# LANL-Bioinformatics/PCRamp

Hardware: AMD Instinct MI355X
Metric: primer-pair x target amplification evals/sec (higher is better)
Workload: dtype u32

## Files before the change

pcramp_amd/csrc/pcr_device.hip:

```cpp
#include <hip/hip_runtime.h>
#include <cstring>
#include <rocprim/device/device_radix_sort.hpp>

#include <stdint.h>
#include <string.h>
#include <math.h>
#include <stdlib.h>
#include <string>
#include <vector>
#include <chrono>
#include <algorithm>
#include <unordered_map>
#include <type_traits>
#include <thread>
#include <mutex>
#include <condition_variable>
#include <functional>
#include <memory>

#include "../../include/pcramp_hip.h"
#include "pcr_host.hpp"

using pcrhost::Planes;

// ... 1188 lines not shown
		const bool vec_ok = ((uintptr_t)d_fr % 16 == 0) && ((uintptr_t)d_rf % 16 == 0) && (bits_bytes % 16 == 0);
		if(!vec_ok){
			HIP_TRY(hipMemsetAsync(d_fr, 0, bits_bytes, ctx->stream));
			HIP_TRY(hipMemsetAsync(d_rf, 0, bits_bytes, ctx->stream));
		}
		if((rc = vec_ok ? st.ship(d_fr, bits_bytes, d_rf, bits_bytes) : st.ship()) != PCR_OK) return rc;
	}
	timer.next(5);
	const uint32_t mask_words = (2*n_pairs + 31)/32;
	if((rc = ctx->mask.ensure((size_t)S.n_slots*mask_words)) != PCR_OK) return rc;
	if((rc = ctx->status.ensure(1)) != PCR_OK) return rc;
	const bool dev_n = S.n_touched == N_TOUCHED_UNKNOWN;
	const uint32_t *n_dev = dev_n ? S.ctrl.p + 3 : nullptr;
	const uint32_t n_t = dev_n ? 0u : S.n_touched, n_db = n_t*S.db_cap;
	const unsigned threads = dev_n ? 256 : 128;
	const unsigned grid = dev_n ? (unsigned)std::min<uint64_t>(((uint64_t)S.n*S.db_cap + threads - 1)/threads, 1024) : (n_db + threads - 1)/threads;
	const unsigned mgrid = dev_n ? std::min<unsigned>((S.n + MATCH_WAVES - 1)/MATCH_WAVES, 1024u) : (n_t + MATCH_WAVES - 1)/MATCH_WAVES;
	hipLaunchKernelGGL(k_match, dim3(std::max(mgrid, 1u)), dim3(64*MATCH_WAVES), 0, ctx->stream, S.db.p, n_t, n_dev, S.db_cap,
		S.touched.p, S.d_seg_hi, ctx->d_oligos, 2*n_pairs, mask_words, ctx->mask.p, ctx->status.p,
		prestaged ? fa->pub_counters : (const uint32_t *)nullptr, prestaged ? ctx->mail_dev + (fa->pub_seq % pcr_ctx::MAIL_RING) : (pcr_ctx::Mail *)nullptr,
		prestaged ? fa->pub_seq : 0u);
	HIP_TRY(hipGetLastError());
	hipLaunchKernelGGL(k_pair, dim3(grid), dim3(threads), 0, ctx->stream, S.db.p, n_db, n_dev, S.db_cap, S.touched.p, S.d_seg_hi, ctx->mask.p,
		mask_words, ctx->d_oligos, n_pairs, S.planes.p, S.d_blk_off.p, S.d_len.p, S.d_active.p, a->amp_min, a->amp_max,
		a->ident_threshold, a->use_taq_mama, d_fr, d_rf, words, ctx->status.p);
	HIP_TRY(hipGetLastError());
	return PCR_OK;
}

template<int NSLOT, int KLO>
int launch_scan2_nw(pcr_ctx *ctx, SeqSet &S, uint32_t nw, uint32_t group0, uint32_t n_groups, uint32_t gw, uint32_t ncand, const HitSink &sink,
	const uint32_t *d_tab, const uint32_t *d_bias, const uint32_t *tile_ids, uint32_t n_tiles, const uint32_t *orient_ids)
{
#define SCAN2_ARGS S.nib.p, S.planes.p, S.valid_d(), S.d_blk_off.p, S.d_len.p, S.d_active.p, S.tile_seq.p, S.tile_pos0.p, \
	d_tab, d_bias, group0, gw, tile_ids, orient_ids, ctx->d_cand_fwd, ctx->d_cand_rc, ctx->d_cand_floor, ncand, sink
	const dim3 grid(n_tiles, n_groups), block(SCAN2_THREADS);
	switch(nw){
		case 1: hipLaunchKernelGGL((k_scan2<1, NSLOT, KLO>), grid, block, 0, ctx->stream, SCAN2_ARGS); break;
		case 2: hipLaunchKernelGGL((k_scan2<2, NSLOT, KLO>), grid, block, 0, ctx->stream, SCAN2_ARGS); break;
		case 3: hipLaunchKernelGGL((k_scan2<3, NSLOT, KLO>), grid, block, 0, ctx->stream, SCAN2_ARGS); break;
		case 4: hipLaunchKernelGGL((k_scan2<4, NSLOT, KLO>), grid, block, 0, ctx->stream, SCAN2_ARGS); break;
		case 5: hipLaunchKernelGGL((k_scan2<5, NSLOT, KLO>), grid, block, 0, ctx->stream, SCAN2_ARGS); break;
		case 6: hipLaunchKernelGGL((k_scan2<6, NSLOT, KLO>), grid, block, 0, ctx->stream, SCAN2_ARGS); break;
		case 7: hipLaunchKernelGGL((k_scan2<7, NSLOT, KLO>), grid, block, 0, ctx->stream, SCAN2_ARGS); break;
		default: hipLaunchKernelGGL((k_scan2<8, NSLOT, KLO>), grid, block, 0, ctx->stream, SCAN2_ARGS); break;
	}
#undef SCAN2_ARGS
// ... 1001 lines not shown
					if(ctx->debug_log) fprintf(stderr, "[pcramp] k_seed: %d workgroups per CU x %u CUs\n", per_cu, ctx->n_cu);
#define SEED_ARGS S.tb_d(), S.planes.p, S.valid_d(), S.d_blk_off.p, S.d_nblk_real.p, S.d_len.p, S.d_active.p, S.tile_seq.p, S.tile_pos0.p, \
	S.tile_degen.p, S.n_tiles, ST, ctx->d_cand_fwd, ctx->d_cand_rc, ctx->d_cand_floor, ncand, IA, sgrid.x, sink
					if(cand_lds) hipLaunchKernelGGL(k_seed<true>, fgrid, sblock, dyn, ctx->stream, SEED_ARGS);
					else hipLaunchKernelGGL(k_seed<false>, fgrid, sblock, dyn, ctx->stream, SEED_ARGS);
#undef SEED_ARGS
					HIP_TRY(hipGetLastError());
					if(need_seedset && (rc = launch_scan2(ctx, S, tab_seedset, ncand, sink, d_tab_seedset, d_bias_seedset, S.degen_tiles.p,
						S.n_degen_tiles, d_map_seedset)) != PCR_OK) return rc;
				}
			}
			scan_prof.finish();
		}
		if(n_live && !irr_fused){
			const unsigned irr_grid = (n_live + IRR_THREADS*IRR_PER_LANE - 1)/(IRR_THREADS*IRR_PER_LANE);
			hipLaunchKernelGGL(k_scan_irr, dim3(irr_grid), dim3(IRR_THREADS), 0, ctx->stream, S.irr.p, S.irr_perm.p, n_live,
				S.d_active.p, ctx->d_cand_fwd, ctx->d_cand_floor, ncand, sink);
			HIP_TRY(hipGetLastError());
		}
		if(async && fa && fa->staged && (cap == POST_CAP || cap == 128 || cap == 256) && 2*fa->n_pairs <= 32*POST_MASK_WORDS){
			++ctx->mail_seq;
			const uint64_t bw = (S.n + 63)/64;
#define POST_ARGS ctx->hits.p, d_seq_count, ctx->best.p, ncand, S.planes.p, S.d_blk_off.p, S.irr.p, S.irr_off.p, S.db.p, S.d_seg_hi, d_counters, ctx->epoch, S.n, \
	fa->d_oligos, fa->n_pairs, (2*fa->n_pairs + 31)/32, S.d_len.p, S.d_active.p, fa->a->amp_min, fa->a->amp_max, \
	fa->a->ident_threshold, fa->a->use_taq_mama, fa->d_fr, fa->d_rf, bw, ctx->mail_dev + (ctx->mail_seq % pcr_ctx::MAIL_RING), ctx->mail_seq
			if(cap == POST_CAP){
				static const int post_waves = getenv("PCRAMP_POST_WAVES") ? atoi(getenv("PCRAMP_POST_WAVES")) : 8;
				if(post_waves == 16) hipLaunchKernelGGL(k_post<16>, dim3((S.n + 15)/16), dim3(1024), 0, ctx->stream, POST_ARGS);
				else if(post_waves == 4) hipLaunchKernelGGL(k_post<4>, dim3((S.n + 3)/4), dim3(256), 0, ctx->stream, POST_ARGS);
				else hipLaunchKernelGGL(k_post<8>, dim3((S.n + 7)/8), dim3(512), 0, ctx->stream, POST_ARGS);
				S.ctrl_clean = true; S.touched_from_seg = true;
			}
			else if(cap == 128) hipLaunchKernelGGL((k_post_big<128, 4>), dim3((S.n + 3)/4), dim3(256), 0, ctx->stream, POST_ARGS);
			else hipLaunchKernelGGL((k_post_big<256, 4>), dim3((S.n + 3)/4), dim3(256), 0, ctx->stream, POST_ARGS);
#undef POST_ARGS
			HIP_TRY(hipGetLastError());
			fa->posted = true;
			S.db_cap = cap; S.n_slots = n_slots;
			S.n_touched = N_TOUCHED_UNKNOWN; S.n_entries = 1; S.have_db = true; S.touched_built = false;
			return PCR_OK;
		}
		hipLaunchKernelGGL(k_touched, dim3((S.n + 255)/256), dim3(256), 0, ctx->stream, d_seq_count, S.n, d_counters, S.touched.p);
		HIP_TRY(hipGetLastError());
		S.touched_built = true;
		uint32_t np2 = 1; while(np2 < cap) np2 <<= 1;
#define FIN_ARGS ctx->hits.p, d_seq_count, cap, ctx->best.p, ncand, S.planes.p, S.d_blk_off.p, S.irr.p, S.irr_off.p, S.db.p, S.d_seg_hi, \
	d_counters, ctx->epoch, S.touched.p
// ... 397 lines not shown
```

pcramp_amd/csrc/pcr_entry_sw_thermo.inc:

```
namespace {

int word_codes(const Planes &w, uint8_t *codes)
{
	const int len = pcrhost::planes_size(w), start = pcrhost::planes_start(w);
	for(int k = 0;k < 32;++k) codes[k] = (k < len && start + k < 32) ? (uint8_t)pcrhost::planes_nibble(w, start + k) : 0;
	return len;
}

void pair_queries(const pcr_pair *pairs, uint32_t n_pairs, std::vector<uint8_t> &q, std::vector<uint8_t> &ql, std::vector<BgPairDev> &bp)
{
	q.assign((size_t)n_pairs*4*32, 0); ql.assign((size_t)n_pairs*4, 0); bp.assign(n_pairs, BgPairDev());
	for(uint32_t p = 0;p < n_pairs;++p){
		const Planes F = pcrhost::planes_of_word(pairs[p].f.w), R = pcrhost::planes_of_word(pairs[p].r.w);
		const Planes o[4] = {F, pcrhost::planes_revcomp(F), R, pcrhost::planes_revcomp(R)};
		uint8_t last[4][2];
		for(int l = 0;l < 4;++l){
			ql[(size_t)p*4 + l] = (uint8_t)word_codes(o[l], &q[((size_t)p*4 + l)*32]);
			const int stop = pcrhost::planes_stop(o[l]);
			last[l][0] = (stop >= 1) ? (uint8_t)pcrhost::planes_nibble(o[l], stop - 1) : 0;
			last[l][1] = (stop >= 0) ? (uint8_t)pcrhost::planes_nibble(o[l], stop) : 0;
		}
		BgPairDev b;
		float f_norm = 2.0f*(unsigned)pcrhost::planes_size(F), r_norm = 2.0f*(unsigned)pcrhost::planes_size(R);
		if(f_norm > 0.0f) f_norm = 1.0f/f_norm;
// ... 200 lines not shown
	int rc;
	const float thr2 = collect_threshold*collect_threshold;
	std::vector<OligoDev> ol(2*(size_t)n_pairs);
	for(uint32_t i = 0;i < n_pairs;++i){ fill_oligo(ol[2*i], pairs[i].f.w, thr2); fill_oligo(ol[2*i + 1], pairs[i].r.w, thr2); }
	if((rc = ctx->oligos.ensure(ol.size())) != PCR_OK) return rc;
	HIP_TRY(hipMemcpyAsync(ctx->oligos.p, ol.data(), ol.size()*sizeof(OligoDev), hipMemcpyHostToDevice, ctx->stream));
	HIP_TRY(hipStreamSynchronize(ctx->stream));
	const uint32_t mask_words = (2*n_pairs + 31)/32;
	if((rc = ctx->mask.ensure((size_t)S.n_slots*mask_words)) != PCR_OK) return rc;
	if((rc = ctx->status.ensure(1)) != PCR_OK) return rc;
	if((rc = ctx->counters.ensure(4)) != PCR_OK) return rc;
	const unsigned threads = 128;
	const uint32_t n_db = S.n_touched*S.db_cap;
	const unsigned grid = (n_db + threads - 1)/threads;
	hipLaunchKernelGGL(k_match, dim3((S.n_touched + MATCH_WAVES - 1)/MATCH_WAVES), dim3(64*MATCH_WAVES), 0, ctx->stream, S.db.p, S.n_touched, (const uint32_t *)nullptr, S.db_cap,
		S.touched.p, S.d_seg_hi, ctx->oligos.p, 2*n_pairs, mask_words, ctx->mask.p, (uint32_t *)nullptr, (const uint32_t *)nullptr, (pcr_ctx::Mail *)nullptr, 0u);
	HIP_TRY(hipGetLastError());
	uint32_t n_amp = 0, status = 0;
	for(int attempt = 0;;++attempt){
		if((rc = ctx->amp_recs.ensure(ctx->amp_cap)) != PCR_OK) return rc;
		HIP_TRY(hipMemsetAsync(ctx->counters.p, 0, 4*sizeof(uint32_t), ctx->stream));
		HIP_TRY(hipMemsetAsync(ctx->status.p, 0, sizeof(uint32_t), ctx->stream));
		hipLaunchKernelGGL(k_pair_emit, dim3(grid), dim3(threads), 0, ctx->stream, S.db.p, n_db, S.db_cap, S.touched.p, S.d_seg_hi, ctx->mask.p, mask_words,
			ctx->oligos.p, n_pairs, S.planes.p, S.d_blk_off.p, S.d_len.p, S.d_active.p, amp_min, amp_max,
			ctx->amp_recs.p, (uint32_t)ctx->amp_cap, ctx->counters.p, ctx->status.p);
		HIP_TRY(hipGetLastError());
		HIP_TRY(hipMemcpyAsync(&n_amp, ctx->counters.p, sizeof(uint32_t), hipMemcpyDeviceToHost, ctx->stream));
		HIP_TRY(hipMemcpyAsync(&status, ctx->status.p, sizeof(uint32_t), hipMemcpyDeviceToHost, ctx->stream));
		HIP_TRY(hipStreamSynchronize(ctx->stream));
		if(n_amp <= ctx->amp_cap) break;
		if(attempt >= 4 || n_amp > (1u << 29)){ g_err = "candidate amplicon list does not fit"; return PCR_ERR_CAPACITY; }
		ctx->amp_cap = (size_t)n_amp + (n_amp >> 3);
	}
	if(status & 1u){ g_err = "Sequence::has_split: range is out of bounds"; return PCR_ERR_RANGE; }
	*n_amp_out = n_amp;
	return PCR_OK;
}

static int background_match_ordered(pcr_ctx *ctx, SeqSet &S, const pcr_pair *pairs, uint32_t n_pairs, const pcr_background_args *args, uint64_t *bits)
{
	const uint64_t words = (S.n + 63)/64;
	const size_t total = (size_t)n_pairs*words;
	int rc;
	uint32_t n_amp = 0;
	if((rc = candidate_amplicons(ctx, S, pairs, n_pairs, args->collect_threshold, args->amp_min, args->amp_max, &n_amp)) != PCR_OK) return rc;
	if((rc = upload_pair_queries(ctx, pairs, n_pairs)) != PCR_OK) return rc;
	if((rc = ctx->bits_fr.ensure(total)) != PCR_OK) return rc;
// ... 496 lines not shown
```

pcramp_amd/csrc/pcr_screen.inc:

```
__device__ __forceinline__ bool db_slot(uint32_t g, uint32_t n, uint32_t cap, const uint32_t *__restrict__ touched,
	const uint32_t *__restrict__ seg_hi, uint32_t &slot)
{
	if(g >= n) return false;
	const uint32_t seq = touched[g/cap];
	slot = seq*cap + g % cap;
	return slot < seg_hi[seq];
}

constexpr int MATCH_WAVES = 4;
__global__ __launch_bounds__(64*MATCH_WAVES) void k_match(const DevEntry *__restrict__ db, uint32_t n_touched, const uint32_t *__restrict__ n_touched_dev, uint32_t cap,
	const uint32_t *__restrict__ touched, const uint32_t *__restrict__ seg_hi, const OligoDev *__restrict__ oligos, uint32_t n_oligo,
	uint32_t mask_words, uint32_t *__restrict__ mask, uint32_t *__restrict__ status,
	const uint32_t *__restrict__ pub_counters, PassMail *pub_mail, uint32_t pub_seq)
{
	if(blockIdx.x == 0 && threadIdx.x == 0 && status) status[0] = 0;
	if(pub_mail && blockIdx.x == 0 && threadIdx.x < 64){
		if(threadIdx.x < 4) pub_mail->counters[threadIdx.x] = pub_counters[threadIdx.x];
		__threadfence_system();
		__builtin_amdgcn_wave_barrier();
		if(threadIdx.x == 0) __hip_atomic_store((uint32_t *)&pub_mail->seq, pub_seq, __ATOMIC_RELEASE, __HIP_MEMORY_SCOPE_SYSTEM);
	}
	if(n_touched_dev) n_touched = *n_touched_dev;
	const uint32_t lane = threadIdx.x & 63u, sub = lane >> 5, ol = lane & 31u;
	for(uint32_t t_idx = blockIdx.x*MATCH_WAVES + (threadIdx.x >> 6);t_idx < n_touched;t_idx += gridDim.x*MATCH_WAVES){
// ... 56 lines not shown
			const float corr = fminf(1.0f, c_taq_mama[16*(4*taq_idx(t2) + taq_idx(t1)) + (4*taq_idx(o.p2) + taq_idx(o.p1))]);
			id = __fmul_rn(id, corr);
		}
	}
	return id;
}

__device__ bool has_split(const uint4 *__restrict__ planes, uint64_t base, int32_t start, int32_t n)
{
	int32_t pos = start;
	const int32_t end = start + n;
	while(pos < end){
		const uint32_t b = (uint32_t)pos >> 5, sh = (uint32_t)pos & 31;
		const uint4 v = planes[base + b];
		uint32_t nz = (v.x | v.y | v.z | v.w) >> sh;
		const int32_t span = min(32 - (int32_t)sh, end - pos);
		const uint32_t want = (span == 32) ? 0xFFFFFFFFu : ((1u << span) - 1u);
		if((nz & want) != want) return true;
		pos += span;
	}
	return false;
}

__global__ void k_pair(const DevEntry *__restrict__ db, uint32_t n, const uint32_t *__restrict__ n_touched_dev, uint32_t cap, const uint32_t *__restrict__ touched,
	const uint32_t *__restrict__ seg_hi, const uint32_t *__restrict__ mask, uint32_t mask_words, const OligoDev *__restrict__ oligos, uint32_t n_pairs,
	const uint4 *__restrict__ planes, const uint64_t *__restrict__ blk_off, const uint64_t *__restrict__ len,
	const uint8_t *__restrict__ active, int32_t amp_min, int32_t amp_max, float ident_thr, int use_taq,
	uint64_t *__restrict__ bits_fr, uint64_t *__restrict__ bits_rf, uint64_t bit_words, uint32_t *__restrict__ status)
{
	if(n_touched_dev) n = (*n_touched_dev)*cap;
	for(uint32_t t = blockIdx.x*blockDim.x + threadIdx.x;t < n;t += gridDim.x*blockDim.x){
	uint32_t i;
	if(!db_slot(t, n, cap, touched, seg_hi, i)) continue;
	const DevEntry ei = db[i];
	if(ei.strand != 1) continue;
	if(!active[ei.seq]) continue;
	const uint32_t hi = seg_hi[ei.seq];
	const int32_t L = (int32_t)len[ei.seq];
	const uint64_t base = blk_off[ei.seq];
	for(uint32_t j = i + 1;j < hi;++j){
		const DevEntry ej = db[j];
		if(ej.loc - ei.loc > amp_max + 128) break;
		if(ej.strand != 2) continue;
		for(uint32_t w = 0;w < mask_words;++w){
			const uint32_t mi = mask[(size_t)i*mask_words + w], mj = mask[(size_t)j*mask_words + w];
			uint32_t fr = mi & (mj >> 1) & 0x55555555u;
			uint32_t rf = (mi >> 1) & mj & 0x55555555u;
			uint32_t any = fr | rf;
			while(any){
				const uint32_t bit = __ffs(any) - 1;
				any &= any - 1;
				const uint32_t pair = (w*32 + bit) >> 1;
				if(pair >= n_pairs) break;
				const OligoDev F = oligos[2*pair], R = oligos[2*pair + 1];
				for(int orient = 0;orient < 2;++orient){
					if(!(((orient == 0) ? fr : rf) >> bit & 1u)) continue;
					const OligoDev &P = (orient == 0) ? F : R;
					const OligoDev &M = (orient == 0) ? R : F;
					if(ei.loc + P.stop >= ej.loc - M.stop) continue;
					int32_t amp_start = ei.loc + P.start;
					const int32_t amp_stop = min(ej.loc - M.start, L - 1);
					int32_t amp_len = amp_stop - amp_start + 1;
					if(amp_len < amp_min || amp_len > amp_max) continue;
					if(amp_start < 0){ amp_len += amp_start; amp_start = 0; }
					if(amp_len < 0 || amp_start + amp_len > L){ atomicOr(status, 1u); continue; }
					if(has_split(planes, base, amp_start, amp_len)) continue;
					const float f = identity(F, (orient == 0) ? ei.w : ej.w, use_taq);
					const float r = identity(R, (orient == 0) ? ej.w : ei.w, use_taq);
					if(sqrtf(__fmul_rn(f, r)) >= ident_thr){
						uint64_t *dst = (orient == 0) ? bits_fr : bits_rf;
						atomicOr((unsigned long long *)&dst[(size_t)pair*bit_words + (ei.seq >> 6)], 1ull << (ei.seq & 63));
					}
				}
			}
		}
	}
	}
}

__global__ void k_pair_moves(const DevEntry *__restrict__ db, uint32_t n, uint32_t cap, const uint32_t *__restrict__ touched,
	const uint32_t *__restrict__ seg_hi, const uint32_t *__restrict__ mask, const OligoDev *__restrict__ base ,
	const OligoDev *__restrict__ variants, uint32_t n_variants, int side,
	const uint4 *__restrict__ planes, const uint64_t *__restrict__ blk_off, const uint64_t *__restrict__ len,
	const uint8_t *__restrict__ active, const uint8_t *__restrict__ has_eos, int32_t amp_min, int32_t amp_max, float ident_thr, int use_taq,
	uint64_t *__restrict__ bits_fr, uint64_t *__restrict__ bits_rf, uint64_t bit_words, uint32_t *__restrict__ status)
{
	const uint32_t t = blockIdx.x*blockDim.x + threadIdx.x;
	uint32_t e;
	if(!db_slot(t, n, cap, touched, seg_hi, e)) return;
// ... 102 lines not shown
			if(iloc + P.stop >= jloc - M.stop) continue;
			int32_t amp_start = iloc + P.start;
			const int32_t amp_stop = min(jloc - M.start, L - 1);
			int32_t amp_len = amp_stop - amp_start + 1;
			if(amp_len < amp_min || amp_len > amp_max) continue;
			if(amp_start < 0){ amp_len += amp_start; amp_start = 0; }
			if(amp_len < 0 || amp_start + amp_len > L){ atomicOr(status, 1u); continue; }
			if(eos && has_split(planes, blk_base, amp_start, amp_len)) continue;
			best = fmaxf(best, r.id);
		}
		if(best < 0.0f) continue;
		uint64_t *dst = (orient == 0) ? bits_fr : bits_rf;
		const uint64_t bit = 1ull << (seq & 63);
		for(uint32_t v = 0;v < n_variants;++v){
			const float var = identity(variants[v], ee.w, use_taq);
			const float f = (side == 0) ? var : best, r2 = (side == 0) ? best : var;
			if(sqrtf(__fmul_rn(f, r2)) >= ident_thr)
				atomicOr((unsigned long long *)&dst[(size_t)v*bit_words + (seq >> 6)], bit);
		}
	}
}

constexpr uint32_t POST_CAP = 64, POST_MASK_WORDS = 4;
struct PostEnt { Planes w; int32_t loc; uint32_t strand; };
template<int POST_WAVES>
struct PostShared {
	OligoDev ol[32*POST_MASK_WORDS];
	uint64_t keys[POST_WAVES][POST_CAP]; PostEnt ent[POST_WAVES][POST_CAP]; uint32_t msk[POST_WAVES][POST_CAP][POST_MASK_WORDS];
};

template<int POST_WAVES>
__global__ __launch_bounds__(64*POST_WAVES) void k_post(const Hit *__restrict__ hits, uint32_t *__restrict__ seq_count,
	const uint32_t *__restrict__ best, uint32_t ncand, const uint4 *__restrict__ planes, const uint64_t *__restrict__ blk_off,
	const IrrDev *__restrict__ irr, const uint32_t *__restrict__ irr_off, DevEntry *__restrict__ db, uint32_t *__restrict__ seg_hi,
	uint32_t *__restrict__ counters, uint32_t epoch, uint32_t n_seq,
	const OligoDev *__restrict__ oligos, uint32_t n_pairs, uint32_t mask_words,
	const uint64_t *__restrict__ len, const uint8_t *__restrict__ active, int32_t amp_min, int32_t amp_max, float ident_thr, int use_taq,
	uint64_t *__restrict__ bits_fr, uint64_t *__restrict__ bits_rf, uint64_t bit_words, PassMail *pub_mail, uint32_t pub_seq)
{
	__shared__ PostShared<POST_WAVES> sh;
	const uint32_t wave = threadIdx.x >> 6, lane = threadIdx.x & 63u;
	if(pub_mail && blockIdx.x == 0 && wave == 0){
		if(lane < 4) pub_mail->counters[lane] = (lane == 3) ? N_TOUCHED_UNKNOWN_DEV : counters[lane];
		__threadfence_system();
		__builtin_amdgcn_wave_barrier();
		if(lane == 0) __hip_atomic_store((uint32_t *)&pub_mail->seq, pub_seq, __ATOMIC_RELEASE, __HIP_MEMORY_SCOPE_SYSTEM);
	}
	if(blockIdx.x == 0 && wave == 0 && lane < 4) counters[lane] = 0;
	const uint32_t seq = blockIdx.x*POST_WAVES + wave;
	const uint32_t n_raw = (seq < n_seq) ? seq_count[seq] : 0u;
	const uint32_t n = min(n_raw, POST_CAP);
	if(seq < n_seq && lane == 0){
		if(n_raw) seq_count[seq] = 0;
		else seg_hi[seq] = 0;
	}
	const uint32_t seq_c = min(seq, n_seq - 1u);
	const uint64_t base = blk_off[seq_c];
	const int32_t L = (int32_t)len[seq_c];
	const uint32_t is_active = active[seq_c];
	if(__syncthreads_or((int)n)){
		const uint32_t nw = 2*n_pairs*(uint32_t)(sizeof(OligoDev)/4);
		for(uint32_t i = threadIdx.x;i < nw;i += 64*POST_WAVES) ((uint32_t *)sh.ol)[i] = ((const uint32_t *)oligos)[i];
		__syncthreads();
	}
	if(n == 0) return;
	uint64_t *keys = sh.keys[wave];
	PostEnt *ent = sh.ent[wave];
	uint64_t k = ~0ull;
	if(lane < n){
		const Hit h = hits[(size_t)seq*POST_CAP + lane];
		if(((epoch << 8) | h.cnt) == best[(size_t)seq*ncand + h.cand]) k = h.key;
	}
	keys[lane] = k;
	wave_sync();
	uint32_t np2 = 1; while(np2 < n) np2 <<= 1;
	for(uint32_t kk = 2;kk <= np2;kk <<= 1){
		for(uint32_t j = kk >> 1;j > 0;j >>= 1){
			const uint32_t l = lane ^ j;
			if(l > lane && l < np2){
				const uint64_t a = keys[lane], b = keys[l];
				const bool up = ((lane & kk) == 0);
				if((a > b) == up){ keys[lane] = b; keys[l] = a; }
			}
			wave_sync();
		}
	}
	k = keys[lane];
	const bool distinct = k != ~0ull && (lane == 0 || keys[lane - 1] != k);
	const uint64_t dmask = __ballot(distinct);
	const uint32_t run = (uint32_t)__builtin_popcountll(dmask);
	const uint32_t rank = (uint32_t)__builtin_popcountll(dmask & ((1ull << lane) - 1ull));
	if(lane == 0) seg_hi[seq] = seq*POST_CAP + run;
	if(distinct){
		DevEntry e;
		materialise_entry_at(k, planes, base, irr, irr_off, e);
// ... 3 lines not shown
	}
	wave_sync();
	if(n_pairs == 0) return;
	const uint32_t n_oligo = 2*n_pairs;
	PostEnt me; me.w.a = me.w.c = me.w.g = me.w.t = 0; me.loc = 0; me.strand = 0;
	if(lane < run) me = ent[lane];
	for(uint32_t g = 0;2*g < mask_words;++g){
		const uint32_t o = g*64 + lane;
		Planes m; m.a = m.c = m.g = m.t = 0; uint32_t fl = 0xFFFFFFFFu;
		if(o < n_oligo){ m = sh.ol[o].m; fl = sh.ol[o].floor2; }
		for(uint32_t e = 0;e < run;++e){
			const Planes w = ent[e].w;
			const uint32_t cnt = __popc((w.a & m.a) | (w.c & m.c) | (w.g & m.g) | (w.t & m.t));
			const uint64_t bal = __ballot(cnt >= fl);
			if(lane == 0){
				sh.msk[wave][e][2*g] = (uint32_t)bal;
				if(2*g + 1 < mask_words) sh.msk[wave][e][2*g + 1] = (uint32_t)(bal >> 32);
			}
		}
	}
	wave_sync();
	if(lane >= run || me.strand != 1 || !is_active) return;
	for(uint32_t j = lane + 1;j < run;++j){
		const PostEnt ej = ent[j];
		if(ej.loc - me.loc > amp_max + 128) break;
		if(ej.strand != 2) continue;
		for(uint32_t w = 0;w < mask_words;++w){
			const uint32_t mi = sh.msk[wave][lane][w], mj = sh.msk[wave][j][w];
			uint32_t fr = mi & (mj >> 1) & 0x55555555u;
			uint32_t rf = (mi >> 1) & mj & 0x55555555u;
			uint32_t any = fr | rf;
			while(any){
				const uint32_t bit = __ffs(any) - 1;
				any &= any - 1;
				const uint32_t pair = (w*32 + bit) >> 1;
				if(pair >= n_pairs) break;
				const OligoDev F = sh.ol[2*pair], R = sh.ol[2*pair + 1];
				for(int orient = 0;orient < 2;++orient){
					if(!(((orient == 0) ? fr : rf) >> bit & 1u)) continue;
					const OligoDev &P = (orient == 0) ? F : R;
					const OligoDev &M = (orient == 0) ? R : F;
					if(me.loc + P.stop >= ej.loc - M.stop) continue;
					int32_t amp_start = me.loc + P.start;
					const int32_t amp_stop = min(ej.loc - M.start, L - 1);
					int32_t amp_len = amp_stop - amp_start + 1;
					if(amp_len < amp_min || amp_len > amp_max) continue;
					if(amp_start < 0){ amp_len += amp_start; amp_start = 0; }
					if(amp_len < 0 || amp_start + amp_len > L){ atomicOr(&counters[1], 1u); continue; }
					if(has_split(planes, base, amp_start, amp_len)) continue;
					const float f = identity(F, (orient == 0) ? me.w : ej.w, use_taq);
					const float r = identity(R, (orient == 0) ? ej.w : me.w, use_taq);
					if(sqrtf(__fmul_rn(f, r)) >= ident_thr){
						uint64_t *dst = (orient == 0) ? bits_fr : bits_rf;
						atomicOr((unsigned long long *)&dst[(size_t)pair*bit_words + (seq >> 6)], 1ull << (seq & 63));
					}
				}
			}
		}
	}
}

template<uint32_t CAP, int WAVES>
struct PostSharedBig {
	OligoDev ol[32*POST_MASK_WORDS];
	uint64_t keys[WAVES][CAP]; DevEntry ent[WAVES][CAP]; uint32_t msk[WAVES][CAP][POST_MASK_WORDS]; uint32_t part[WAVES][64];
};

template<uint32_t CAP, int WAVES>
__global__ __launch_bounds__(64*WAVES) void k_post_big(const Hit *__restrict__ hits, const uint32_t *__restrict__ seq_count,
	const uint32_t *__restrict__ best, uint32_t ncand, const uint4 *__restrict__ planes, const uint64_t *__restrict__ blk_off,
	const IrrDev *__restrict__ irr, const uint32_t *__restrict__ irr_off, DevEntry *__restrict__ db, uint32_t *__restrict__ seg_hi,
	uint32_t *__restrict__ counters, uint32_t epoch, uint32_t n_seq,
	const OligoDev *__restrict__ oligos, uint32_t n_pairs, uint32_t mask_words,
	const uint64_t *__restrict__ len, const uint8_t *__restrict__ active, int32_t amp_min, int32_t amp_max, float ident_thr, int use_taq,
	uint64_t *__restrict__ bits_fr, uint64_t *__restrict__ bits_rf, uint64_t bit_words, PassMail *pub_mail, uint32_t pub_seq)
{
	__shared__ PostSharedBig<CAP, WAVES> sh;
	const uint32_t wave = threadIdx.x >> 6, lane = threadIdx.x & 63u;
	if(pub_mail && blockIdx.x == 0 && wave == 0){
		if(lane < 4) pub_mail->counters[lane] = (lane == 3) ? N_TOUCHED_UNKNOWN_DEV : counters[lane];
		__threadfence_system();
		__builtin_amdgcn_wave_barrier();
		if(lane == 0) __hip_atomic_store((uint32_t *)&pub_mail->seq, pub_seq, __ATOMIC_RELEASE, __HIP_MEMORY_SCOPE_SYSTEM);
	}
	const uint32_t seq = blockIdx.x*WAVES + wave;
	const uint32_t n = (seq < n_seq) ? min(seq_count[seq], CAP) : 0u;
	if(__syncthreads_or((int)n)){
		const uint32_t nw = 2*n_pairs*(uint32_t)(sizeof(OligoDev)/4);
		for(uint32_t i = threadIdx.x;i < nw;i += 64*WAVES) ((uint32_t *)sh.ol)[i] = ((const uint32_t *)oligos)[i];
		__syncthreads();
	}
	if(n == 0) return;
	uint64_t *keys = sh.keys[wave];
	DevEntry *ent = sh.ent[wave];
	uint32_t *part = sh.part[wave];
	uint32_t np2 = 1; while(np2 < n) np2 <<= 1;
	for(uint32_t i = lane;i < np2;i += 64){
// ... 41 lines not shown
		}
	}
	wave_sync();
	if(n_pairs == 0) return;
	const uint32_t n_oligo = 2*n_pairs;
	for(uint32_t e = lane;e < run;e += 64){
		const DevEntry me = ent[e];
		for(uint32_t mw = 0;mw < mask_words;++mw){
			uint32_t bits = 0;
			const uint32_t o_end = min(n_oligo, (mw + 1)*32);
#pragma unroll 4
			for(uint32_t o = mw*32;o < o_end;++o){
				const Planes m = sh.ol[o].m;
				const uint32_t c = __popc((me.w.a & m.a) | (me.w.c & m.c) | (me.w.g & m.g) | (me.w.t & m.t));
				bits |= (uint32_t)(c >= sh.ol[o].floor2) << (o & 31);
			}
			sh.msk[wave][e][mw] = bits;
		}
	}
	wave_sync();
	if(!active[seq]) return;
	const int32_t L = (int32_t)len[seq];
	const uint64_t base = blk_off[seq];
	for(uint32_t i = lane;i < run;i += 64){
		const DevEntry me = ent[i];
		if(me.strand != 1) continue;
		for(uint32_t j = i + 1;j < run;++j){
			const DevEntry ej = ent[j];
			if(ej.loc - me.loc > amp_max + 128) break;
			if(ej.strand != 2) continue;
			for(uint32_t w = 0;w < mask_words;++w){
				const uint32_t mi = sh.msk[wave][i][w], mj = sh.msk[wave][j][w];
				uint32_t fr = mi & (mj >> 1) & 0x55555555u;
				uint32_t rf = (mi >> 1) & mj & 0x55555555u;
				uint32_t any = fr | rf;
				while(any){
					const uint32_t bit = __ffs(any) - 1;
					any &= any - 1;
					const uint32_t pair = (w*32 + bit) >> 1;
					if(pair >= n_pairs) break;
					const OligoDev F = sh.ol[2*pair], R = sh.ol[2*pair + 1];
					for(int orient = 0;orient < 2;++orient){
						if(!(((orient == 0) ? fr : rf) >> bit & 1u)) continue;
						const OligoDev &P = (orient == 0) ? F : R;
						const OligoDev &M = (orient == 0) ? R : F;
						if(me.loc + P.stop >= ej.loc - M.stop) continue;
						int32_t amp_start = me.loc + P.start;
						const int32_t amp_stop = min(ej.loc - M.start, L - 1);
						int32_t amp_len = amp_stop - amp_start + 1;
						if(amp_len < amp_min || amp_len > amp_max) continue;
						if(amp_start < 0){ amp_len += amp_start; amp_start = 0; }
						if(amp_len < 0 || amp_start + amp_len > L){ atomicOr(&counters[1], 1u); continue; }
						if(has_split(planes, base, amp_start, amp_len)) continue;
						const float f = identity(F, (orient == 0) ? me.w : ej.w, use_taq);
						const float r = identity(R, (orient == 0) ? ej.w : me.w, use_taq);
						if(sqrtf(__fmul_rn(f, r)) >= ident_thr){
							uint64_t *dst = (orient == 0) ? bits_fr : bits_rf;
							atomicOr((unsigned long long *)&dst[(size_t)pair*bit_words + (seq >> 6)], 1ull << (seq & 63));
						}
					}
				}
			}
		}
	}
}
```

pcramp_amd/csrc/pcr_sw.inc:

```

struct SwOut { int16_t score, q_start, q_stop, t_start, t_stop; uint8_t last1, last2, valid, pad; };

struct SwJob { uint32_t q; uint32_t tlen; uint64_t t_off; };

struct SwCell { int M, Iq, It, Msi, Msj, Iqsi, Iqsj, Itsi, Itsj; };

__device__ __forceinline__ uint32_t pack16(int a, int b) { return ((uint32_t)a & 0xFFFFu) | ((uint32_t)b << 16); }
__device__ __forceinline__ int lo16(uint32_t v) { return (int)(int16_t)(v & 0xFFFFu); }
__device__ __forceinline__ int hi16(uint32_t v) { return (int)(int16_t)(v >> 16); }

constexpr int SW_THREADS = 256;
constexpr int SW_GAP_OPEN = -5, SW_GAP_EXT = -2, SW_MATCH = 2, SW_MISMATCH = -3;

template<bool COORDS, class TCode>
__device__ __forceinline__ void sw_lane(bool have_job, int qlen, int tlen, int qi, TCode tcode, SwOut &r)
{
	const int i = threadIdx.x & 31;
	SwCell C = {0, SW_GAP_OPEN, SW_GAP_OPEN, i + 1, 0, 0, 0, 0, 0};
	SwCell A = {0, SW_GAP_OPEN, SW_GAP_OPEN, 0, 0, 0, 0, 0, 0};
	int tcur = 0;
	int chunk = 0;
	int best = -32768, best_j = 0, best_si = 0, best_sj = 0;

	const int n_steps = (qlen > 0 && tlen > 0) ? (qlen + tlen - 1) : 0;
// ... 135 lines not shown
	uint32_t code = 0;
	if(k < len && start + k < 32) code = nibble_at(w, start + k);
	codes[(size_t)e*32 + k] = (uint8_t)code;
	if(k == 0) lens[e] = (uint8_t)len;
}

__global__ void k_seq_codes(const uint32_t *__restrict__ nib, const uint64_t *__restrict__ blk_off, const uint64_t *__restrict__ len,
	const uint64_t *__restrict__ code_off, uint32_t n_seq, uint8_t *__restrict__ codes)
{
	const uint32_t s = blockIdx.y;
	if(s >= n_seq) return;
	const uint64_t L = len[s];
	for(uint64_t p = (uint64_t)blockIdx.x*blockDim.x + threadIdx.x;p < L;p += (uint64_t)gridDim.x*blockDim.x){
		const uint32_t w = nib[blk_off[s]*4 + (p >> 3)];
		codes[code_off[s] + p] = (uint8_t)((w >> ((p & 7)*4)) & 0xF);
	}
}

struct AmpRec { uint32_t pair, seq, f_entry, r_entry; };

__global__ void k_pair_emit(const DevEntry *__restrict__ db, uint32_t n, uint32_t db_cap, const uint32_t *__restrict__ touched, const uint32_t *__restrict__ seg_hi,
	const uint32_t *__restrict__ mask, uint32_t mask_words, const OligoDev *__restrict__ oligos, uint32_t n_pairs,
	const uint4 *__restrict__ planes, const uint64_t *__restrict__ blk_off, const uint64_t *__restrict__ len,
	const uint8_t *__restrict__ active, int32_t amp_min, int32_t amp_max,
	AmpRec *__restrict__ recs, uint32_t cap, uint32_t *__restrict__ counter, uint32_t *__restrict__ status)
{
	const uint32_t t = blockIdx.x*blockDim.x + threadIdx.x;
	uint32_t i;
	if(!db_slot(t, n, db_cap, touched, seg_hi, i)) return;
	const DevEntry ei = db[i];
	if(ei.strand != 1) return;
	if(!active[ei.seq]) return;
	const uint32_t hi = seg_hi[ei.seq];
	const int32_t L = (int32_t)len[ei.seq];
	const uint64_t base = blk_off[ei.seq];
	for(uint32_t j = i + 1;j < hi;++j){
		const DevEntry ej = db[j];
		if(ej.loc - ei.loc > amp_max + 128) break;
		if(ej.strand != 2) continue;
		for(uint32_t w = 0;w < mask_words;++w){
			const uint32_t mi = mask[(size_t)i*mask_words + w], mj = mask[(size_t)j*mask_words + w];
			const uint32_t fr = mi & (mj >> 1) & 0x55555555u;
			const uint32_t rf = (mi >> 1) & mj & 0x55555555u;
			uint32_t any = fr | rf;
			while(any){
				const uint32_t bit = __ffs(any) - 1;
				any &= any - 1;
				const uint32_t pair = (w*32 + bit) >> 1;
				if(pair >= n_pairs) break;
				const OligoDev F = oligos[2*pair], R = oligos[2*pair + 1];
				for(int orient = 0;orient < 2;++orient){
					if(!(((orient == 0) ? fr : rf) >> bit & 1u)) continue;
					const OligoDev &P = (orient == 0) ? F : R;
					const OligoDev &M = (orient == 0) ? R : F;
					if(ei.loc + P.stop >= ej.loc - M.stop) continue;
					int32_t amp_start = ei.loc + P.start;
					const int32_t amp_stop = min(ej.loc - M.start, L - 1);
					int32_t amp_len = amp_stop - amp_start + 1;
					if(amp_len < amp_min || amp_len > amp_max) continue;
					if(amp_start < 0){ amp_len += amp_start; amp_start = 0; }
					if(amp_len < 0 || amp_start + amp_len > L){ atomicOr(status, 1u); continue; }
					if(has_split(planes, base, amp_start, amp_len)) continue;
					const uint32_t k = atomicAdd(counter, 1u);
					if(k < cap){
						AmpRec r; r.pair = pair; r.seq = ei.seq;
						r.f_entry = (orient == 0) ? i : j;
						r.r_entry = (orient == 0) ? j : i;
						recs[k] = r;
					}
				}
			}
		}
	}
}

constexpr int BGE_WAVES = 4, BGE_LIST = 64, BGE_MW = 8, BGE_SUB = 16;
template<int STAGE>
__global__ __launch_bounds__(64*BGE_WAVES) void k_bg_emit(const DevEntry *__restrict__ db, uint32_t n_touched, uint32_t db_cap, const uint32_t *__restrict__ touched,
	const uint32_t *__restrict__ seg_hi, const uint32_t *__restrict__ mask, uint32_t mask_words, const OligoDev *__restrict__ oligos, uint32_t n_pairs,
	const uint4 *__restrict__ planes, const uint64_t *__restrict__ blk_off, const uint64_t *__restrict__ len,
	const uint8_t *__restrict__ active, const uint8_t *__restrict__ has_eos, int32_t amp_min, int32_t amp_max,
	AmpRec *__restrict__ recs, uint32_t sub_cap , uint32_t *__restrict__ sub_count , uint32_t *__restrict__ status)
{
	constexpr bool STAGED = STAGE > 0;
	extern __shared__ uint32_t bge_geom[];
// ... 341 lines not shown
```

Measured before the change: 19.79 billion.

## Skip split checks for sequences without separators and streamline k_post

Adds a per-sequence has_eos flag and skips the has_split plane scan in k_pair, k_post, k_post_big and k_pair_emit when a sequence contains no separator. In k_post, a batched split check loads several plane blocks at once. The oligo table is prefetched into registers before the barrier. The best-candidate lookup in global memory is replaced by a wave-level readlane comparison over hits. It also adds a waves-per-EU attribute, a readfirstlane on the wave index, and a profiling script. The risks are correctness if has_eos is not populated, and a changed tie rule for hit selection.

```diff
diff --git a/pcramp_amd/csrc/pcr_device.hip b/pcramp_amd/csrc/pcr_device.hip
--- a/pcramp_amd/csrc/pcr_device.hip
+++ b/pcramp_amd/csrc/pcr_device.hip
@@ -1234,7 +1234,7 @@
 		prestaged ? fa->pub_seq : 0u);
 	HIP_TRY(hipGetLastError());
 	hipLaunchKernelGGL(k_pair, dim3(grid), dim3(threads), 0, ctx->stream, S.db.p, n_db, n_dev, S.db_cap, S.touched.p, S.d_seg_hi, ctx->mask.p,
-		mask_words, ctx->d_oligos, n_pairs, S.planes.p, S.d_blk_off.p, S.d_len.p, S.d_active.p, a->amp_min, a->amp_max,
+		mask_words, ctx->d_oligos, n_pairs, S.planes.p, S.d_blk_off.p, S.d_len.p, S.d_active.p, S.d_has_eos.p, a->amp_min, a->amp_max,
 		a->ident_threshold, a->use_taq_mama, d_fr, d_rf, words, ctx->status.p);
 	HIP_TRY(hipGetLastError());
 	return PCR_OK;
@@ -2282,7 +2282,7 @@
 			++ctx->mail_seq;
 			const uint64_t bw = (S.n + 63)/64;
 #define POST_ARGS ctx->hits.p, d_seq_count, ctx->best.p, ncand, S.planes.p, S.d_blk_off.p, S.irr.p, S.irr_off.p, S.db.p, S.d_seg_hi, d_counters, ctx->epoch, S.n, \
-	fa->d_oligos, fa->n_pairs, (2*fa->n_pairs + 31)/32, S.d_len.p, S.d_active.p, fa->a->amp_min, fa->a->amp_max, \
+	fa->d_oligos, fa->n_pairs, (2*fa->n_pairs + 31)/32, S.d_len.p, S.d_active.p, S.d_has_eos.p, fa->a->amp_min, fa->a->amp_max, \
 	fa->a->ident_threshold, fa->a->use_taq_mama, fa->d_fr, fa->d_rf, bw, ctx->mail_dev + (ctx->mail_seq % pcr_ctx::MAIL_RING), ctx->mail_seq
 			if(cap == POST_CAP){
 				static const int post_waves = getenv("PCRAMP_POST_WAVES") ? atoi(getenv("PCRAMP_POST_WAVES")) : 8;
diff --git a/pcramp_amd/csrc/pcr_entry_sw_thermo.inc b/pcramp_amd/csrc/pcr_entry_sw_thermo.inc
--- a/pcramp_amd/csrc/pcr_entry_sw_thermo.inc
+++ b/pcramp_amd/csrc/pcr_entry_sw_thermo.inc
@@ -246,7 +246,7 @@
 		HIP_TRY(hipMemsetAsync(ctx->counters.p, 0, 4*sizeof(uint32_t), ctx->stream));
 		HIP_TRY(hipMemsetAsync(ctx->status.p, 0, sizeof(uint32_t), ctx->stream));
 		hipLaunchKernelGGL(k_pair_emit, dim3(grid), dim3(threads), 0, ctx->stream, S.db.p, n_db, S.db_cap, S.touched.p, S.d_seg_hi, ctx->mask.p, mask_words,
-			ctx->oligos.p, n_pairs, S.planes.p, S.d_blk_off.p, S.d_len.p, S.d_active.p, amp_min, amp_max,
+			ctx->oligos.p, n_pairs, S.planes.p, S.d_blk_off.p, S.d_len.p, S.d_active.p, S.d_has_eos.p, amp_min, amp_max,
 			ctx->amp_recs.p, (uint32_t)ctx->amp_cap, ctx->counters.p, ctx->status.p);
 		HIP_TRY(hipGetLastError());
 		HIP_TRY(hipMemcpyAsync(&n_amp, ctx->counters.p, sizeof(uint32_t), hipMemcpyDeviceToHost, ctx->stream));
diff --git a/pcramp_amd/csrc/pcr_screen.inc b/pcramp_amd/csrc/pcr_screen.inc
--- a/pcramp_amd/csrc/pcr_screen.inc
+++ b/pcramp_amd/csrc/pcr_screen.inc
@@ -102,10 +102,36 @@
 	return false;
 }
 
+template<int NB>
+__device__ __forceinline__ bool has_split_batched(const uint4 *__restrict__ planes, uint64_t base, int32_t start, int32_t n)
+{
+	if(n <= 0) return false;
+	const int32_t end = start + n;
+	const uint32_t b_last = (uint32_t)(end - 1) >> 5;
+	for(uint32_t b0 = (uint32_t)start >> 5;b0 <= b_last;b0 += NB){
+		uint32_t nz[NB];
+#pragma unroll
+		for(int i = 0;i < NB;++i){
+			const uint4 v = planes[base + min(b0 + (uint32_t)i, b_last)];
+			nz[i] = v.x | v.y | v.z | v.w;
+		}
+		bool cut = false;
+#pragma unroll
+		for(int i = 0;i < NB;++i){
+			const int32_t p0 = (int32_t)(min(b0 + (uint32_t)i, b_last) << 5);
+			const int32_t lo = max(start, p0) - p0, hi = min(end, p0 + 32) - p0;
+			const uint32_t want = ((hi == 32) ? 0xFFFFFFFFu : ((1u << hi) - 1u)) & ~((1u << lo) - 1u);
+			cut |= (nz[i] & want) != want;
+		}
+		if(cut) return true;
+	}
+	return false;
+}
+
 __global__ void k_pair(const DevEntry *__restrict__ db, uint32_t n, const uint32_t *__restrict__ n_touched_dev, uint32_t cap, const uint32_t *__restrict__ touched,
 	const uint32_t *__restrict__ seg_hi, const uint32_t *__restrict__ mask, uint32_t mask_words, const OligoDev *__restrict__ oligos, uint32_t n_pairs,
 	const uint4 *__restrict__ planes, const uint64_t *__restrict__ blk_off, const uint64_t *__restrict__ len,
-	const uint8_t *__restrict__ active, int32_t amp_min, int32_t amp_max, float ident_thr, int use_taq,
+	const uint8_t *__restrict__ active, const uint8_t *__restrict__ has_eos, int32_t amp_min, int32_t amp_max, float ident_thr, int use_taq,
 	uint64_t *__restrict__ bits_fr, uint64_t *__restrict__ bits_rf, uint64_t bit_words, uint32_t *__restrict__ status)
 {
 	if(n_touched_dev) n = (*n_touched_dev)*cap;
@@ -118,6 +144,7 @@
 	const uint32_t hi = seg_hi[ei.seq];
 	const int32_t L = (int32_t)len[ei.seq];
 	const uint64_t base = blk_off[ei.seq];
+	const bool eos = has_eos[ei.seq] != 0;
 	for(uint32_t j = i + 1;j < hi;++j){
 		const DevEntry ej = db[j];
 		if(ej.loc - ei.loc > amp_max + 128) break;
@@ -144,7 +171,7 @@
 					if(amp_len < amp_min || amp_len > amp_max) continue;
 					if(amp_start < 0){ amp_len += amp_start; amp_start = 0; }
 					if(amp_len < 0 || amp_start + amp_len > L){ atomicOr(status, 1u); continue; }
-					if(has_split(planes, base, amp_start, amp_len)) continue;
+					if(eos && has_split(planes, base, amp_start, amp_len)) continue;
 					const float f = identity(F, (orient == 0) ? ei.w : ej.w, use_taq);
 					const float r = identity(R, (orient == 0) ? ej.w : ei.w, use_taq);
 					if(sqrtf(__fmul_rn(f, r)) >= ident_thr){
@@ -293,6 +320,8 @@
 }
 
 constexpr uint32_t POST_CAP = 64, POST_MASK_WORDS = 4;
+constexpr int POST_SPLIT_BATCH = 4;
+#define POST_WAVES_PER_EU __attribute__((amdgpu_waves_per_eu(8, 8)))
 struct PostEnt { Planes w; int32_t loc; uint32_t strand; };
 template<int POST_WAVES>
 struct PostShared {
@@ -301,16 +330,16 @@
 };
 
 template<int POST_WAVES>
-__global__ __launch_bounds__(64*POST_WAVES) void k_post(const Hit *__restrict__ hits, uint32_t *__restrict__ seq_count,
+__global__ __launch_bounds__(64*POST_WAVES) POST_WAVES_PER_EU void k_post(const Hit *__restrict__ hits, uint32_t *__restrict__ seq_count,
 	const uint32_t *__restrict__ best, uint32_t ncand, const uint4 *__restrict__ planes, const uint64_t *__restrict__ blk_off,
 	const IrrDev *__restrict__ irr, const uint32_t *__restrict__ irr_off, DevEntry *__restrict__ db, uint32_t *__restrict__ seg_hi,
 	uint32_t *__restrict__ counters, uint32_t epoch, uint32_t n_seq,
 	const OligoDev *__restrict__ oligos, uint32_t n_pairs, uint32_t mask_words,
-	const uint64_t *__restrict__ len, const uint8_t *__restrict__ active, int32_t amp_min, int32_t amp_max, float ident_thr, int use_taq,
+	const uint64_t *__restrict__ len, const uint8_t *__restrict__ active, const uint8_t *__restrict__ has_eos, int32_t amp_min, int32_t amp_max, float ident_thr, int use_taq,
 	uint64_t *__restrict__ bits_fr, uint64_t *__restrict__ bits_rf, uint64_t bit_words, PassMail *pub_mail, uint32_t pub_seq)
 {
 	__shared__ PostShared<POST_WAVES> sh;
-	const uint32_t wave = threadIdx.x >> 6, lane = threadIdx.x & 63u;
+	const uint32_t wave = (uint32_t)__builtin_amdgcn_readfirstlane((int)(threadIdx.x >> 6)), lane = threadIdx.x & 63u;
 	if(pub_mail && blockIdx.x == 0 && wave == 0){
 		if(lane < 4) pub_mail->counters[lane] = (lane == 3) ? N_TOUCHED_UNKNOWN_DEV : counters[lane];
 		__threadfence_system();
@@ -329,19 +358,35 @@
 	const uint64_t base = blk_off[seq_c];
 	const int32_t L = (int32_t)len[seq_c];
 	const uint32_t is_active = active[seq_c];
+	const bool eos = has_eos[seq_c] != 0;
+	constexpr uint32_t OL_WORDS = 32*POST_MASK_WORDS*(uint32_t)(sizeof(OligoDev)/4), OL_REGS = (OL_WORDS + 64*POST_WAVES - 1)/(64*POST_WAVES);
+	const uint32_t nw = 2*n_pairs*(uint32_t)(sizeof(OligoDev)/4);
+	uint32_t olw[OL_REGS];
+#pragma unroll
+	for(uint32_t r = 0;r < OL_REGS;++r){
+		const uint32_t i = r*64*POST_WAVES + threadIdx.x;
+		olw[r] = (i < nw) ? ((const uint32_t *)oligos)[i] : 0u;
+	}
+	Hit h; h.key = ~0ull; h.cand = 0; h.cnt = 0;
+	if(lane < n) h = hits[(size_t)seq*POST_CAP + lane];
 	if(__syncthreads_or((int)n)){
-		const uint32_t nw = 2*n_pairs*(uint32_t)(sizeof(OligoDev)/4);
-		for(uint32_t i = threadIdx.x;i < nw;i += 64*POST_WAVES) ((uint32_t *)sh.ol)[i] = ((const uint32_t *)oligos)[i];
+#pragma unroll
+		for(uint32_t r = 0;r < OL_REGS;++r){
+			const uint32_t i = r*64*POST_WAVES + threadIdx.x;
+			if(i < nw) ((uint32_t *)sh.ol)[i] = olw[r];
+		}
 		__syncthreads();
 	}
 	if(n == 0) return;
 	uint64_t *keys = sh.keys[wave];
 	PostEnt *ent = sh.ent[wave];
-	uint64_t k = ~0ull;
-	if(lane < n){
-		const Hit h = hits[(size_t)seq*POST_CAP + lane];
-		if(((epoch << 8) | h.cnt) == best[(size_t)seq*ncand + h.cand]) k = h.key;
-	}
+	bool top = lane < n;
+	const uint32_t n_u = (uint32_t)__builtin_amdgcn_readfirstlane((int)n);
+	for(uint32_t e = 0;e < n_u;++e){
+		const uint32_t e_cand = (uint32_t)__builtin_amdgcn_readlane((int)h.cand, (int)e), e_cnt = (uint32_t)__builtin_amdgcn_readlane((int)h.cnt, (int)e);
+		if(e_cand == h.cand && e_cnt > h.cnt) top = false;
+	}
+	uint64_t k = top ? h.key : ~0ull;
 	keys[lane] = k;
 	wave_sync();
 	uint32_t np2 = 1; while(np2 < n) np2 <<= 1;
@@ -391,9 +436,9 @@
 	wave_sync();
 	if(lane >= run || me.strand != 1 || !is_active) return;
 	for(uint32_t j = lane + 1;j < run;++j){
-		const PostEnt ej = ent[j];
-		if(ej.loc - me.loc > amp_max + 128) break;
-		if(ej.strand != 2) continue;
+		const int32_t ej_loc = ent[j].loc;
+		if(ej_loc - me.loc > amp_max + 128) break;
+		if(ent[j].strand != 2) continue;
 		for(uint32_t w = 0;w < mask_words;++w){
 			const uint32_t mi = sh.msk[wave][lane][w], mj = sh.msk[wave][j][w];
 			uint32_t fr = mi & (mj >> 1) & 0x55555555u;
@@ -404,21 +449,23 @@
 				any &= any - 1;
 				const uint32_t pair = (w*32 + bit) >> 1;
 				if(pair >= n_pairs) break;
-				const OligoDev F = sh.ol[2*pair], R = sh.ol[2*pair + 1];
+				const OligoDev *const F = &sh.ol[2*pair], *const R = F + 1;
 				for(int orient = 0;orient < 2;++orient){
 					if(!(((orient == 0) ? fr : rf) >> bit & 1u)) continue;
-					const OligoDev &P = (orient == 0) ? F : R;
-					const OligoDev &M = (orient == 0) ? R : F;
-					if(me.loc + P.stop >= ej.loc - M.stop) continue;
-					int32_t amp_start = me.loc + P.start;
-					const int32_t amp_stop = min(ej.loc - M.start, L - 1);
+					const OligoDev *const P = (orient == 0) ? F : R;
+					const OligoDev *const M = (orient == 0) ? R : F;
+					if(me.loc + P->stop >= ej_loc - M->stop) continue;
+					int32_t amp_start = me.loc + P->start;
+					const int32_t amp_stop = min(ej_loc - M->start, L - 1);
 					int32_t amp_len = amp_stop - amp_start + 1;
 					if(amp_len < amp_min || amp_len > amp_max) continue;
 					if(amp_start < 0){ amp_len += amp_start; amp_start = 0; }
 					if(amp_len < 0 || amp_start + amp_len > L){ atomicOr(&counters[1], 1u); continue; }
-					if(has_split(planes, base, amp_start, amp_len)) continue;
-					const float f = identity(F, (orient == 0) ? me.w : ej.w, use_taq);
-					const float r = identity(R, (orient == 0) ? ej.w : me.w, use_taq);
+					if(eos && has_split_batched<POST_SPLIT_BATCH>(planes, base, amp_start, amp_len)) continue;
+					const Planes wj = ent[j].w;
+					const OligoDev Fo = *F, Ro = *R;
+					const float f = identity(Fo, (orient == 0) ? me.w : wj, use_taq);
+					const float r = identity(Ro, (orient == 0) ? wj : me.w, use_taq);
 					if(sqrtf(__fmul_rn(f, r)) >= ident_thr){
 						uint64_t *dst = (orient == 0) ? bits_fr : bits_rf;
 						atomicOr((unsigned long long *)&dst[(size_t)pair*bit_words + (seq >> 6)], 1ull << (seq & 63));
@@ -441,7 +488,7 @@
 	const IrrDev *__restrict__ irr, const uint32_t *__restrict__ irr_off, DevEntry *__restrict__ db, uint32_t *__restrict__ seg_hi,
 	uint32_t *__restrict__ counters, uint32_t epoch, uint32_t n_seq,
 	const OligoDev *__restrict__ oligos, uint32_t n_pairs, uint32_t mask_words,
-	const uint64_t *__restrict__ len, const uint8_t *__restrict__ active, int32_t amp_min, int32_t amp_max, float ident_thr, int use_taq,
+	const uint64_t *__restrict__ len, const uint8_t *__restrict__ active, const uint8_t *__restrict__ has_eos, int32_t amp_min, int32_t amp_max, float ident_thr, int use_taq,
 	uint64_t *__restrict__ bits_fr, uint64_t *__restrict__ bits_rf, uint64_t bit_words, PassMail *pub_mail, uint32_t pub_seq)
 {
 	__shared__ PostSharedBig<CAP, WAVES> sh;
@@ -529,6 +576,7 @@
 	if(!active[seq]) return;
 	const int32_t L = (int32_t)len[seq];
 	const uint64_t base = blk_off[seq];
+	const bool eos = has_eos[seq] != 0;
 	for(uint32_t i = lane;i < run;i += 64){
 		const DevEntry me = ent[i];
 		if(me.strand != 1) continue;
@@ -558,7 +606,7 @@
 						if(amp_len < amp_min || amp_len > amp_max) continue;
 						if(amp_start < 0){ amp_len += amp_start; amp_start = 0; }
 						if(amp_len < 0 || amp_start + amp_len > L){ atomicOr(&counters[1], 1u); continue; }
-						if(has_split(planes, base, amp_start, amp_len)) continue;
+						if(eos && has_split(planes, base, amp_start, amp_len)) continue;
 						const float f = identity(F, (orient == 0) ? me.w : ej.w, use_taq);
 						const float r = identity(R, (orient == 0) ? ej.w : me.w, use_taq);
 						if(sqrtf(__fmul_rn(f, r)) >= ident_thr){
diff --git a/pcramp_amd/csrc/pcr_sw.inc b/pcramp_amd/csrc/pcr_sw.inc
--- a/pcramp_amd/csrc/pcr_sw.inc
+++ b/pcramp_amd/csrc/pcr_sw.inc
@@ -181,7 +181,7 @@
 __global__ void k_pair_emit(const DevEntry *__restrict__ db, uint32_t n, uint32_t db_cap, const uint32_t *__restrict__ touched, const uint32_t *__restrict__ seg_hi,
 	const uint32_t *__restrict__ mask, uint32_t mask_words, const OligoDev *__restrict__ oligos, uint32_t n_pairs,
 	const uint4 *__restrict__ planes, const uint64_t *__restrict__ blk_off, const uint64_t *__restrict__ len,
-	const uint8_t *__restrict__ active, int32_t amp_min, int32_t amp_max,
+	const uint8_t *__restrict__ active, const uint8_t *__restrict__ has_eos, int32_t amp_min, int32_t amp_max,
 	AmpRec *__restrict__ recs, uint32_t cap, uint32_t *__restrict__ counter, uint32_t *__restrict__ status)
 {
 	const uint32_t t = blockIdx.x*blockDim.x + threadIdx.x;
@@ -193,6 +193,7 @@
 	const uint32_t hi = seg_hi[ei.seq];
 	const int32_t L = (int32_t)len[ei.seq];
 	const uint64_t base = blk_off[ei.seq];
+	const bool eos = has_eos[ei.seq] != 0;
 	for(uint32_t j = i + 1;j < hi;++j){
 		const DevEntry ej = db[j];
 		if(ej.loc - ei.loc > amp_max + 128) break;
@@ -219,7 +220,7 @@
 					if(amp_len < amp_min || amp_len > amp_max) continue;
 					if(amp_start < 0){ amp_len += amp_start; amp_start = 0; }
 					if(amp_len < 0 || amp_start + amp_len > L){ atomicOr(status, 1u); continue; }
-					if(has_split(planes, base, amp_start, amp_len)) continue;
+					if(eos && has_split(planes, base, amp_start, amp_len)) continue;
 					const uint32_t k = atomicAdd(counter, 1u);
 					if(k < cap){
 						AmpRec r; r.pair = pair; r.seq = ei.seq;
diff --git a/profiles/pass_percentiles.py b/profiles/pass_percentiles.py
--- /dev/null
+++ b/profiles/pass_percentiles.py
@@ -0,0 +1,25 @@
+#!/usr/bin/env python3
+import csv, glob, os, sys
+import numpy as np
+
+d = sys.argv[1]
+f = max(glob.glob(d + "/*/*_kernel_trace.csv"), key=os.path.getmtime)
+ev = []
+for r in csv.DictReader(open(f)):
+    n = r["Kernel_Name"]
+    k = "seed" if "k_seed3" in n else "post" if "k_post" in n else None
+    if k:
+        ev.append((int(r["Start_Timestamp"]), int(r["End_Timestamp"]), k))
+ev.sort()
+seed, gap1, post, gap2, period = [], [], [], [], []
+for i in range(len(ev) - 2):
+    a, b, c = ev[i], ev[i + 1], ev[i + 2]
+    if a[2] == "seed" and b[2] == "post" and c[2] == "seed":
+        seed.append(a[1] - a[0]); gap1.append(b[0] - a[1]); post.append(b[1] - b[0]); gap2.append(c[0] - b[1]); period.append(c[0] - a[0])
+print("%d consecutive passes; microseconds" % len(seed))
+print("| | median | p10 | p90 | mean |")
+print("|---|---|---|---|---|")
+for name, v in (("`k_seed3` (start to end)", seed), ("end of `k_seed3` to start of `k_post`", gap1), ("`k_post`", post),
+                ("end of `k_post` to start of the next `k_seed3`", gap2), ("pass period (start to start)", period)):
+    v = np.array(v) / 1e3
+    print("| %s | %.2f | %.2f | %.2f | %.2f |" % (name, np.median(v), np.percentile(v, 10), np.percentile(v, 90), v.mean()))
```

After: 20.67 billion, median of 6. 4.4% higher.
